# google/lyra

Hardware: NVIDIA H100
Metric: 20ms-frame encode+decode throughput (frames/s) @16kHz (higher is better)
Workload: dtype f32+i8 (decoder fp32 GEMMs: split tf32 on tensor cores)

## Files before the change

lyra_b200/csrc/kernel_prims.cuh:

```cuda
#pragma once

#include "device_compat.h"
#include "net_params.h"

namespace lyra_b200 {

template <typename T>
__device__ __forceinline__ const T* BlobPtr(const uint8_t* blob, uint32_t off) {
  return reinterpret_cast<const T*>(blob + off);
}

__device__ __forceinline__ float LeakyRelu(float v) { return fmaxf(v, __fmul_rn(v, 0.3f)); }

__device__ __forceinline__ int QuantizeF32(float v, float scale, int zp) {
  int q = (int)roundf(__fdiv_rn(v, scale)) + zp;
  q = q < -128 ? -128 : (q > 127 ? 127 : q);
  return q;
}
__device__ __forceinline__ float DequantizeI8(int q, float scale, int zp) { return __fmul_rn(scale, (float)(q - zp)); }

__device__ __forceinline__ int Mbqm(int x, int qm, int shift) {
  const int left = shift > 0 ? shift : 0, right = shift > 0 ? 0 : -shift;
  const long long ab = (long long)(int)((unsigned)x << left) * (long long)qm;
  const int hi = (int)((ab + (1ll << 30)) >> 31);
// ... 225 lines not shown
    const int tr0 = valid0 ? m0 / S : T_out - 1, tr1 = valid1 ? m1 / S : T_out - 1;
    const int s0 = m0 % S, s1 = m1 % S;
    const int grp = (nt0 * 8) / CoutG;
    const uint32_t* pa0 = A + (size_t)(grp * CinG4) * ldA + (rowA0 + tr0 * row_stride) * S + s0;
    const uint32_t* pa1 = A + (size_t)(grp * CinG4) * ldA + (rowA0 + tr1 * row_stride) * S + s1;
    const uint2* wp = Wf + (size_t)nt0 * 32 + lane;
    const size_t ks_stride = (size_t)NTILES * 32;
    int acc[NTW][4];
#pragma unroll
    for (int j = 0; j < NTW; ++j) { acc[j][0] = 0; acc[j][1] = 0; acc[j][2] = 0; acc[j][3] = 0; }
    uint2 bf[PD][NTW];
#pragma unroll
    for (int p = 0; p < PD; ++p)
      if (p < KS) {
#pragma unroll
        for (int j = 0; j < NTW; ++j) bf[p][j] = __ldg(wp + p * ks_stride + j * 32);
      }
    for (int ks0 = 0; ks0 < KS; ks0 += PD) {
#pragma unroll
      for (int p = 0; p < PD; ++p) {
        const int ks = ks0 + p;
        if (ks < KS) {
          const int kw = ks * 8, tap = kw / CinG4, kw0 = kw - tap * CinG4;
          const size_t off = (size_t)(kw0 + t4) * ldA + tap * S;
          uint32_t a[4];
          a[0] = pa0[off]; a[1] = pa1[off]; a[2] = pa0[off + 4 * (size_t)ldA]; a[3] = pa1[off + 4 * (size_t)ldA];
#pragma unroll
          for (int j = 0; j < NTW; ++j) {
            const uint32_t b[2] = {bf[p][j].x, bf[p][j].y};
            lyra_mma_s8_16x8x32(acc[j], a, b);
          }
          if (ks + PD < KS) {
#pragma unroll
            for (int j = 0; j < NTW; ++j) bf[p][j] = __ldg(wp + (size_t)(ks + PD) * ks_stride + j * 32);
          }
        }
      }
    }
    const bool even = (t4 & 1) == 0;
#pragma unroll
    for (int j = 0; j < NTW; ++j) {
      const int r0 = __shfl_xor_sync(0xffffffffu, even ? acc[j][2] : acc[j][0], 1);
      const int r1 = __shfl_xor_sync(0xffffffffu, even ? acc[j][3] : acc[j][1], 1);
      int out[1][4];
      if (even) { out[0][0] = acc[j][0]; out[0][1] = acc[j][1]; out[0][2] = r0; out[0][3] = r1; }
      else { out[0][0] = r0; out[0][1] = r1; out[0][2] = acc[j][2]; out[0][3] = acc[j][3]; }
      const int n4 = (nt0 + j) * 8 + (t4 >> 1) * 4;
      if (even ? valid0 : valid1) epi(even ? tr0 : tr1, even ? s0 : s1, n4, out);
    }
  }
  __syncthreads();
}

__host__ __device__ constexpr int PadLd(int x) {
  while (!(x % 4 == 0 && (x % 32 == 8 || x % 32 == 24))) ++x;
  return x;
}

__device__ __forceinline__ void SplitTf32(float x, uint32_t& hi, uint32_t& lo) {
  hi = __float_as_uint(x) & 0xffffe000u;
  lo = __float_as_uint(__fsub_rn(x, __uint_as_float(hi)));
}

template <int S, int NT, int WTM, int WTN, bool SYNC_EPI, typename Epi>
__device__ __forceinline__ void GemmTf32Mma(const float* A, int ldA, int rowA0, int row_stride, int ntaps, int CinG,
                                            int groups, int T_out, int N, const float2* __restrict__ Wf, Epi epi) {
  constexpr int PD = 8;
  constexpr int NW = NT / 32;
  const int lane = (int)threadIdx.x & 31, warp = (int)threadIdx.x >> 5, g = lane >> 2, t4 = lane & 3;
  const int M = T_out * S, MT = (M + 15) / 16, MTW = (MT + WTM - 1) / WTM, NTILES = N / 8, NWT = MTW * (NTILES / WTN);
  const int KS = ntaps * CinG / 8, CoutG = N / groups;
  const size_t ks_stride = (size_t)NTILES * 32;
  float acc[WTM][WTN][4];
  int tr[WTM][2], sr[WTM][2];
  bool vr[WTM][2];
  int nt0 = 0;

  auto kloop = [&](int wt) {
    const int mtb = (wt % MTW) * WTM;
    nt0 = (wt / MTW) * WTN;
    const int grp = (nt0 * 8) / CoutG;
    const float* pa[WTM][2];
#pragma unroll
    for (int i = 0; i < WTM; ++i)
#pragma unroll
      for (int h = 0; h < 2; ++h) {
        const int m = (mtb + i) * 16 + g + 8 * h;
        vr[i][h] = m < M;
        tr[i][h] = vr[i][h] ? m / S : T_out - 1;
        sr[i][h] = m % S;
        pa[i][h] = A + (size_t)(grp * CinG) * ldA + (rowA0 + tr[i][h] * row_stride) * S + sr[i][h];
      }
#pragma unroll
    for (int i = 0; i < WTM; ++i)
#pragma unroll
      for (int j = 0; j < WTN; ++j) { acc[i][j][0] = 0.0f; acc[i][j][1] = 0.0f; acc[i][j][2] = 0.0f; acc[i][j][3] = 0.0f; }
    const float2* wp = Wf + (size_t)nt0 * 32 + lane;
    float2 bf[PD][WTN];
#pragma unroll
    for (int p = 0; p < PD; ++p)
      if (p < KS) {
#pragma unroll
        for (int j = 0; j < WTN; ++j) bf[p][j] = __ldg(wp + p * ks_stride + j * 32);
      }
    for (int ks0 = 0; ks0 < KS; ks0 += PD) {
#pragma unroll
// ... 238 lines not shown
```

lyra_b200/csrc/net_kernels.cuh:

```cuda
#pragma once

#include <type_traits>

#include "kernel_prims.cuh"

namespace lyra_b200 {

constexpr int kTileStreams = 8;

struct EncStateA {
  static constexpr int kFirst = 0;
  static constexpr int kRing0 = 48, kRing1 = kRing0 + 64 * 2, kRing2 = kRing1 + 64 * 6;
  static constexpr int kDown0 = kRing2 + 64 * 18;
  static constexpr int kUnits = kDown0 + 64 * 5;
  static constexpr int kT = 20;
};
struct EncStateB {
  static constexpr int kRing0 = 0, kRing1 = 128 * 2, kRing2 = kRing1 + 128 * 6;
  static constexpr int kDown1 = kRing2 + 128 * 18;
  static constexpr int kRingM = kDown1 + 128 * 2;
  static constexpr int kRingQ0 = kRingM + 256 * 2;
  static constexpr int kRingQ1 = kRingQ0 + 64 * 6;
  static constexpr int kDown2 = kRingQ1 + 64 * 18;
  static constexpr int kBott = kDown2 + 64 * 2;
// ... 144 lines not shown
    auto epi2 = [&](int t, int s0, int n0, auto& acc) {
      constexpr int TMx = sizeof(acc) / sizeof(acc[0]), TNx = sizeof(acc[0]) / sizeof(float);
#pragma unroll
      for (int j = 0; j < TNx; ++j) {
        const float b = b2[n0 + j];
        float* o = u + (size_t)(n0 + j) * ldu + (row0u + t) * S + s0;
#pragma unroll
        for (int i = 0; i < TMx; ++i) {
          const float v = __fadd_rn(__fadd_rn(acc[i][j], b), o[i]);
          o[i] = last ? LeakyRelu(v) : v;
        }
      }
    };
    if constexpr (TC)
      GemmTf32Mma<S, NT, WTM, WTN, false>(d, ldd, 0, 1, 1, C / groups2, groups2, T, C, BlobPtr<float2>(blob, p.pw2.wf), epi2);
    else
      GemmF32Tap<S, NT, TM, TN2, KC, WM, false, STG>(d, ldd, 0, 1, 1, C / groups2, groups2, T, C, BlobPtr<float>(blob, p.pw2.w), wbuf, true, after, epi2);
  }
}

template <int S, int NT, int TM, int TN1, int TN2, int WM, int KC, int C, int T, bool TC = false, int LDD = T * S, int WTM = 1, int WTN = 1,
          int STG = kStages>
__device__ __forceinline__ void ResUnitsF32x3(const uint8_t* blob, const ResF32* p3, float* u, int ldu, int row0u, float* d, int groups2,
                                              float* ring0, const int* n18, const int* active, float* wbuf, const WNext& after) {
#pragma unroll 1
  for (int i = 0; i < 3; ++i) {
    const ResF32& p = p3[i];
    const int dil = i == 0 ? 1 : (i == 1 ? 3 : 9);
    float* ring = ring0 + (size_t)(i == 0 ? 0 : (i == 1 ? 2 : 8)) * C * S;
    const WNext nx = i < 2 ? NextF32(BlobPtr<float>(blob, p3[i + 1].pw1.w), KC, C, C, nullptr, STG) : after;
    ResUnitF32<S, NT, TM, TN1, TN2, WM, KC, C, T, 0, TC, LDD, WTM, WTN, STG>(blob, p, u, ldu, row0u, d, groups2, ring, n18, active, wbuf, i == 2, nx,
                                                                       dil);
  }
}

struct RequantLutPack {
  const int* bias;
  const int* mult;
  const int* shift;
  const int8_t* lut;
  int out_zp;
  __device__ __forceinline__ RequantLutPack(const uint8_t* blob, const GemmI8& g, const LReluQ& lr)
      : bias(BlobPtr<int>(blob, g.bias)), mult(BlobPtr<int>(blob, g.mult)), shift(BlobPtr<int>(blob, g.shift)),
        lut(BlobPtr<int8_t>(blob, lr.lut)), out_zp(g.out_zp) {}
  __device__ __forceinline__ uint32_t operator()(const int (&acc)[1][4], int n0) const {
    const RequantP4 rq = LoadRequant4(bias, mult, shift, n0);
    int q[4];
#pragma unroll
    for (int j = 0; j < 4; ++j) q[j] = lut[RequantI8(acc[0][j], rq.b[j], rq.m[j], rq.s[j], out_zp) + 128];
    return PackI8x4(q[0], q[1], q[2], q[3]);
  }
};

template <int S, int NT, int PDI, typename Params>
__device__ __forceinline__ void MixedUnitPw2I8(const uint8_t* blob, const Params& P, const uint32_t* hq, const float* u,
                                               uint32_t* resq, uint32_t* aq, int lda, int row0a) {
  constexpr int LQ2 = PadLd(2 * S), LD2 = 2 * S;
  const int* bias = BlobPtr<int>(blob, P.m_pw2.bias);
  const int* mult = BlobPtr<int>(blob, P.m_pw2.mult);
  const int* shift = BlobPtr<int>(blob, P.m_pw2.shift);
  const int8_t* lut = BlobPtr<int8_t>(blob, P.m_lr2.lut);
  const QuantP dq = P.m_dq, q2 = P.m_q2;
  const int out_zp = P.m_pw2.out_zp;
  GemmI8Mma<S, NT, 4, PDI>(hq, LQ2, 0, 1, 1, 64, 4, 2, 256, BlobPtr<uint2>(blob, P.m_pw2.w),
    [&](int t, int s, int n0, int (&acc)[1][4]) {
      const RequantP4 rq = LoadRequant4(bias, mult, shift, n0);
      int r[4], a[4];
#pragma unroll
      for (int j = 0; j < 4; ++j) {
        const int q = RequantI8(acc[0][j], rq.b[j], rq.m[j], rq.s[j], out_zp);
        const float v = __fadd_rn(DequantizeI8(q, dq.scale, dq.zp), u[(size_t)(n0 + j) * LD2 + t * S + s]);
        r[j] = QuantizeF32(v, q2.scale, q2.zp);
        a[j] = lut[r[j] + 128];
      }
      resq[(size_t)(n0 / 4) * LQ2 + t * S + s] = PackI8x4(r[0], r[1], r[2], r[3]);
      aq[(size_t)(n0 / 4) * lda + (row0a + t) * S + s] = PackI8x4(a[0], a[1], a[2], a[3]);
    });
}

template <int S, int NT, int DIL, int PDI = kI8Pd>
__device__ __forceinline__ void ResUnitI8(const uint8_t* blob, const ResI8& p, uint32_t* aq, int lda, int row0a,
                                          uint32_t* resq, uint32_t* dq8, uint32_t* hq, uint32_t* ring,
                                          const int* n18, const int* active, int dil_rt = DIL) {
  constexpr int T = kResI8Rows, C = 256, LD = PadLd(T * S);
  constexpr int NTW = 4;
  if (n18[S] >= 0) {
    if constexpr (DIL != 0) DwI8RingFast<S, NT, C, T, DIL>(aq, lda, row0a, dq8, LD, blob, p.dw, ring, n18[S], active);
    else if (dil_rt == 3) DwI8RingFast<S, NT, C, T, 3>(aq, lda, row0a, dq8, LD, blob, p.dw, ring, n18[S], active);
    else DwI8RingFast<S, NT, C, T, 9>(aq, lda, row0a, dq8, LD, blob, p.dw, ring, n18[S], active);
  } else {
    DwI8Ring<S, NT>(aq, lda, row0a, dq8, LD, C, T, dil_rt, blob, p.dw, ring, n18, active);
  }
  {
    const RequantLutPack epi(blob, p.pw1, p.lr1);
    GemmI8Mma<S, NT, NTW, PDI>(dq8, LD, 0, 1, 1, C, 1, T, C, BlobPtr<uint2>(blob, p.pw1.w),
      [&](int t, int s, int n0, int (&acc)[1][4]) { hq[(size_t)(n0 / 4) * LD + t * S + s] = epi(acc, n0); });
  }
  {
    const int* bias = BlobPtr<int>(blob, p.pw2.bias);
    const int* mult = BlobPtr<int>(blob, p.pw2.mult);
    const int* shift = BlobPtr<int>(blob, p.pw2.shift);
    const int* l1 = BlobPtr<int>(blob, p.add.lut1);
    const int* l2 = BlobPtr<int>(blob, p.add.lut2);
    const int8_t* lut = BlobPtr<int8_t>(blob, p.lr2.lut);
    const int out_zp = p.pw2.out_zp, m3 = p.add.m3, s3 = p.add.s3, add_zp = p.add.out_zp;
    GemmI8Mma<S, NT, NTW, PDI>(hq, LD, 0, 1, 1, C / 4, 4, T, C, BlobPtr<uint2>(blob, p.pw2.w),
      [&](int t, int s, int n0, int (&acc)[1][4]) {
        const RequantP4 rq = LoadRequant4(bias, mult, shift, n0);
        const size_t ro = (size_t)(n0 / 4) * LD + t * S + s;
        const uint32_t rw = resq[ro];
        int r[4], a[4];
#pragma unroll
        for (int j = 0; j < 4; ++j) {
          const int q = RequantI8(acc[0][j], rq.b[j], rq.m[j], rq.s[j], out_zp);
          r[j] = ClampI8(Mbqm(l1[q + 128] + l2[UnpackI8(rw, j) + 128], m3, s3) + add_zp);
          a[j] = lut[r[j] + 128];
        }
        resq[ro] = PackI8x4(r[0], r[1], r[2], r[3]);
        aq[(size_t)(n0 / 4) * lda + (row0a + t) * S + s] = PackI8x4(a[0], a[1], a[2], a[3]);
      });
  }
}

template <int S, int NT, int PDI = kI8Pd>
__device__ __forceinline__ void ResUnitsI8x2(const uint8_t* blob, const ResI8* p2, uint32_t* aq, int lda, int row0a,
                                             uint32_t* resq, uint32_t* dq8, uint32_t* hq, uint32_t* ring0,
                                             const int* n18, const int* active) {
#pragma unroll 1
  for (int i = 0; i < 2; ++i)
    ResUnitI8<S, NT, 0, PDI>(blob, p2[i], aq, lda, row0a, resq, dq8, hq, ring0 + (size_t)(i ? 64 * 6 : 0) * S, n18, active, i ? 9 : 3);
}

struct EncA {
  static constexpr int S = kTileStreams;
  static constexpr int NT = 320;
  static constexpr int TN = 4;
  static constexpr int kMinBlocks = 2;
  static constexpr int LDU = 25 * S, LDD = 20 * S;
  static constexpr int kStgDown = 5;
  static constexpr int DTM = 8, DTN = 4;
  static constexpr int kSmemU = 0;
  static constexpr int kSmemD = kSmemU + 64 * LDU * 4;
  static constexpr int kSmemW = kSmemD + 64 * LDD * 4;
  static constexpr int kSmemI = kSmemW + kStages * 16 * 64 * 4;
  static constexpr int kSmemBytes = kSmemI + 3 * S * 4 + 16;
  static_assert(391 * S <= 64 * LDD, "first-layer input (368 rows + 23 skew rows) must fit in the d buffer");
};

__global__ void __launch_bounds__(EncA::NT, EncA::kMinBlocks)
EncoderKernelA(const uint8_t* __restrict__ blob, EncoderParams P, TileIo io, const int16_t* __restrict__ pcm,
               float* __restrict__ state, int* __restrict__ n18g, float* __restrict__ mid) {
  using L = EncA;
  constexpr int S = L::S, NT = L::NT;
  unsigned char* smem = LYRA_DYN_SMEM();
  float* u = reinterpret_cast<float*>(smem + L::kSmemU);
  float* d = reinterpret_cast<float*>(smem + L::kSmemD);
  float* wbuf = reinterpret_cast<float*>(smem + L::kSmemW);
  int* slot = reinterpret_cast<int*>(smem + L::kSmemI);
  int* active = slot + S;
  int* n18 = active + S;
  int tile;
  InitWeightPipe<NT>();
  if (!BeginTile<S>(io, n18g, slot, state, EncStateA::kUnits, tile)) return;
  float* st = state + (size_t)tile * EncStateA::kUnits * S;
  const int tid = (int)threadIdx.x;
  IssuePrologue<NT>(wbuf, NextF32(BlobPtr<float>(blob, P.first.w), 16, 64, 64));

  float* X = d;
  BatchedLoop<NT, 2, float>(48 * S, [&](int i) { return st[EncStateA::kFirst * S + i]; },
                            [&](int i, float v) { const int r = i / S; X[(r + (r >> 4)) * S + i % S] = v; });
  BatchedLoop<NT, 8, float>(320 * S,
    [&](int i) { const int s = i / 320, k = i % 320; return active[s] ? (float)pcm[(size_t)slot[s] * 320 + k] * (1.0f / 32768.0f) : 0.0f; },
    [&](int i, float v) { const int s = i / 320, k = i % 320; X[(48 + k + ((48 + k) >> 4)) * S + s] = v; });
  BatchedLoop<NT, 8, float>(64 * 5 * S, [&](int i) { return st[EncStateA::kDown0 * S + i]; },
                            [&](int i, float v) { const int c = i / (5 * S), r = i % (5 * S); u[(size_t)c * L::LDU + r] = v; });
  __syncthreads();
  for (int i = tid; i < 48 * S; i += NT)
    if (active[i % S]) { const int r = 320 + i / S; st[EncStateA::kFirst * S + i] = X[(r + (r >> 4)) * S + i % S]; }
  {
    const float* b = BlobPtr<float>(blob, P.first.bias);
    GemmF32Tap<S, NT, 8, L::TN, 16, 4, true>(X, 0, 0, 17, 64, 1, 1, 20, 64, BlobPtr<float>(blob, P.first.w), wbuf, true,
      NextF32(BlobPtr<float>(blob, P.r0[0].pw1.w), 16, 64, 64),
      [&](int t, int s0, int n0, float (&acc)[8][L::TN]) {
#pragma unroll
        for (int j = 0; j < L::TN; ++j) {
          float* o = u + (size_t)(n0 + j) * L::LDU + (5 + t) * S + s0;
#pragma unroll
          for (int i = 0; i < 8; ++i) o[i] = __fadd_rn(acc[i][j], b[n0 + j]);
        }
      });
  }
  static_assert(EncStateA::kRing1 == EncStateA::kRing0 + 64 * 2 && EncStateA::kRing2 == EncStateA::kRing1 + 64 * 6, "ring blocks back to back");
  ResUnitsF32x3<S, NT, 8, L::TN, L::TN, 4, 16, 64, EncStateA::kT>(blob, P.r0, u, L::LDU, 5, d, 1, st + (size_t)EncStateA::kRing0 * S, n18, active, wbuf,
                                                       NextF32(BlobPtr<float>(blob, P.down0.w), 16, 128, 640, d, L::kStgDown));
  StoreCarriedRows<S, NT, 64, 5>(st, EncStateA::kDown0, u, L::LDU, 20, active);
  {
    const float* b = BlobPtr<float>(blob, P.down0.bias);
    float* out = mid + (size_t)tile * 128 * 4 * S;
    static_assert(L::kStgDown * 16 * 128 * 4 <= 64 * L::LDD * 4, "simpleconv weight ring must fit in d");
    constexpr int DTM = L::DTM, DTN = L::DTN;
    GemmF32Tap<S, NT, DTM, DTN, 16, 4, false, L::kStgDown>(u, L::LDU, 0, 5, 10, 64, 1, 4, 128, BlobPtr<float>(blob, P.down0.w), d, true, NoNext(),
      [&](int t, int s0, int n0, float (&acc)[DTM][DTN]) {
#pragma unroll
        for (int j = 0; j < DTN; ++j) {
          float* o = out + ((size_t)(n0 + j) * 4 + t) * S + s0;
#pragma unroll
          for (int i = 0; i < DTM; ++i) o[i] = __fadd_rn(acc[i][j], b[n0 + j]);
        }
      });
  }
  AdvanceHopCounters<S>(n18g, tile, active, n18);
}

struct EncB {
  static constexpr int S = kTileStreams;
  static constexpr int NT = 256;
  static constexpr int kMinBlocks = 3;
  static constexpr int TM = 8;
  static constexpr int TN = 4;
  static constexpr int WM4 = 4 * S / TM >= 4 ? 4 : 4 * S / TM;
  static constexpr int WM2 = 2 * S / TM >= 4 ? 4 : 2 * S / TM;
  static constexpr int WM1 = 1 * S / TM >= 4 ? 4 : 1 * S / TM;
  static constexpr int LD1 = 6 * S;
  static constexpr int LQ2 = PadLd(2 * S), LQA = PadLd(4 * S), LQB = PadLd(3 * S);
  static constexpr int kRA = 0;
  static constexpr int kRABytes = kMax(kMax(128 * LD1 * 4, 256 * 2 * S * 4), 64 * LQA * 4 + 128 * LQB * 4);
  static constexpr int kRB = kRA + kRABytes;
  static constexpr int kRBBytes = kMax(128 * 4 * S * 4, 256 * 2 * S * 4);
  static constexpr int kRC = kRB + kRBBytes;
  static constexpr int kW = kRC + 64 * LQ2 * 4;
  static constexpr int kStg = 3;
  static constexpr int kWBytes = kMax(kStg * 8 * 256 * 4, 2 * 64 * LQ2 * 4);
  static constexpr int kI8Pd = 4;
  static constexpr int kI = kW + kWBytes;
  static constexpr int kSmemBytes = kI + 3 * S * 4 + 16;
};

__global__ void __launch_bounds__(EncB::NT, EncB::kMinBlocks)
EncoderKernelB(const uint8_t* __restrict__ blob, EncoderParams P, TileIo io, const float* __restrict__ mid,
               float* __restrict__ state, int* __restrict__ n18g, float* __restrict__ features) {
  using L = EncB;
  constexpr int S = L::S, NT = L::NT;
  constexpr int TM = L::TM, TN = L::TN;
  unsigned char* smem = LYRA_DYN_SMEM();
  constexpr int LQ2 = L::LQ2, LQA = L::LQA, LQB = L::LQB;
  float* u1 = reinterpret_cast<float*>(smem + L::kRA);
  float* d2 = reinterpret_cast<float*>(smem + L::kRA);
  uint32_t* aq = reinterpret_cast<uint32_t*>(smem + L::kRA);
  uint32_t* bq = aq + 64 * LQA;
  float* d1 = reinterpret_cast<float*>(smem + L::kRB);
  float* u2 = reinterpret_cast<float*>(smem + L::kRB);
  uint32_t* hq = reinterpret_cast<uint32_t*>(smem + L::kRC);
  float* wbuf = reinterpret_cast<float*>(smem + L::kW);
  uint32_t* dq8 = reinterpret_cast<uint32_t*>(smem + L::kW);
  uint32_t* resq = dq8 + 64 * LQ2;
  int* slot = reinterpret_cast<int*>(smem + L::kI);
  int* active = slot + S;
  int* n18 = active + S;
  int tile;
  InitWeightPipe<NT>();
  if (!BeginTile<S>(io, n18g, slot, state, EncStateB::kUnits, tile)) return;
  float* st = state + (size_t)tile * EncStateB::kUnits * S;
  uint32_t* stw = reinterpret_cast<uint32_t*>(st);
  IssuePrologue<NT>(wbuf, NextF32(BlobPtr<float>(blob, P.r1[0].pw1.w), 16, 128, 128, nullptr, L::kStg));

  {
    const float* in = mid + (size_t)tile * 128 * 4 * S;
    BatchedLoop<NT, 4, float4>(128 * S, [&](int i) { return reinterpret_cast<const float4*>(in)[i]; },
      [&](int i, float4 v) { const int c = i / S, r = (i % S) * 4; *reinterpret_cast<float4*>(u1 + (size_t)c * L::LD1 + 2 * S + r) = v; });
    BatchedLoop<NT, 8, float>(128 * 2 * S, [&](int i) { return st[EncStateB::kDown1 * S + i]; },
      [&](int i, float v) { const int c = i / (2 * S), r = i % (2 * S); u1[(size_t)c * L::LD1 + r] = v; });
  }
  __syncthreads();
  static_assert(EncStateB::kRing1 == EncStateB::kRing0 + 128 * 2 && EncStateB::kRing2 == EncStateB::kRing1 + 128 * 6, "ring blocks back to back");
  ResUnitsF32x3<S, NT, TM, TN, TN, L::WM4, 16, 128, EncStateB::kT1, false, 4 * S, 1, 1, L::kStg>(
      blob, P.r1, u1, L::LD1, 2, d1, 2, st + (size_t)EncStateB::kRing0 * S, n18, active, wbuf,
      NextF32(BlobPtr<float>(blob, P.down1.w), 8, 256, 256, wbuf, L::kStg));
  StoreCarriedRows<S, NT, 128, 2>(st, EncStateB::kDown1, u1, L::LD1, 4, active);
  {
    const float* b = BlobPtr<float>(blob, P.down1.bias);
    GemmF32Tap<S, NT, TM, TN, 8, L::WM2, false, L::kStg>(u1, L::LD1, 0, 2, 4, 64, 2, 2, 256, BlobPtr<float>(blob, P.down1.w), wbuf, true,
      NextF32(BlobPtr<float>(blob, P.m_pw1.w), 8, 256, 256, wbuf, L::kStg),
      [&](int t, int s0, int n0, float (&acc)[TM][TN]) {
#pragma unroll
        for (int j = 0; j < TN; ++j) {
          float* o = u2 + (size_t)(n0 + j) * 2 * S + t * S + s0;
#pragma unroll
          for (int i = 0; i < TM; ++i) o[i] = __fadd_rn(acc[i][j], b[n0 + j]);
        }
      });
  }
  constexpr int LD2 = 2 * S;
  if (n18[S] >= 0)
    DwF32RingFast<S, NT, 256, EncStateB::kT2, 1>(u2, LD2, 0, d2, LD2, BlobPtr<float>(blob, P.m_dw.w), BlobPtr<float>(blob, P.m_dw.bias),
                                    st + (size_t)EncStateB::kRingM * S, n18[S], active);
  else
    DwF32Ring<S, NT>(u2, LD2, 0, d2, LD2, 256, EncStateB::kT2, 1, BlobPtr<float>(blob, P.m_dw.w), BlobPtr<float>(blob, P.m_dw.bias),
                     st + (size_t)EncStateB::kRingM * S, n18, active);
  {
    const float* b = BlobPtr<float>(blob, P.m_pw1.bias);
    const int8_t* lut = BlobPtr<int8_t>(blob, P.m_lr1.lut);
    const QuantP q1 = P.m_q1;
    static_assert(TN == 4, "the epilogue packs one word of four channels per (row, stream)");
    GemmF32Tap<S, NT, TM, TN, 8, L::WM2, false, L::kStg>(d2, LD2, 0, 1, 1, 256, 1, 2, 256, BlobPtr<float>(blob, P.m_pw1.w), wbuf, true,
      NoNext(),
      [&](int t, int s0, int n0, float (&acc)[TM][TN]) {
#pragma unroll
        for (int i = 0; i < TM; ++i) {
          int q[TN];
#pragma unroll
          for (int j = 0; j < TN; ++j) q[j] = lut[QuantizeF32(__fadd_rn(acc[i][j], b[n0 + j]), q1.scale, q1.zp) + 128];
          hq[(size_t)(n0 / 4) * LQ2 + t * S + s0 + i] = PackI8x4(q[0], q[1], q[2], q[3]);
        }
      });
  }
  MixedUnitPw2I8<S, NT, L::kI8Pd>(blob, P, hq, u2, resq, aq, LQA, 2);
  static_assert(EncStateB::kRingQ1 == EncStateB::kRingQ0 + 64 * 6, "ring blocks back to back");
  ResUnitsI8x2<S, NT, L::kI8Pd>(blob, P.q, aq, LQA, 2, resq, dq8, hq, stw + (size_t)EncStateB::kRingQ0 * S, n18, active);
  BatchedLoop<NT, 4, uint32_t>(64 * 2 * S, [&](int i) { return stw[EncStateB::kDown2 * S + i]; },
    [&](int i, uint32_t v) { const int c = i / (2 * S), r = i % (2 * S); aq[(size_t)c * LQA + r] = v; });
  BatchedLoop<NT, 8, uint32_t>(128 * 2 * S, [&](int i) { return stw[EncStateB::kBott * S + i]; },
    [&](int i, uint32_t v) { const int c = i / (2 * S), r = i % (2 * S); bq[(size_t)c * LQB + r] = v; });
  __syncthreads();
  StoreCarriedRows<S, NT, 64, 2>(stw, EncStateB::kDown2, aq, LQA, 2, active);
  {
    const RequantLutPack epi(blob, P.down2, P.down2_lr);
    GemmI8Mma<S, NT, 8, L::kI8Pd>(aq, LQA, 0, 2, 4, 64, 4, 1, 512, BlobPtr<uint2>(blob, P.down2.w),
      [&](int, int s, int n0, int (&acc)[1][4]) { bq[(size_t)(n0 / 4) * LQB + 2 * S + s] = epi(acc, n0); });
  }
  StoreCarriedRows<S, NT, 128, 2>(stw, EncStateB::kBott, bq, LQB, 1, active);
  {
    const int* bias = BlobPtr<int>(blob, P.bott.bias);
    const int* mult = BlobPtr<int>(blob, P.bott.mult);
    const int* shift = BlobPtr<int>(blob, P.bott.shift);
    const QuantP dq = P.out_dq;
    const int out_zp = P.bott.out_zp;
    GemmI8Mma<S, NT, 1, L::kI8Pd>(bq, LQB, 0, 1, 3, 128, 4, 1, 64, BlobPtr<uint2>(blob, P.bott.w),
      [&](int t, int s, int n0, int (&acc)[1][4]) {
        const RequantP4 rq = LoadRequant4(bias, mult, shift, n0);
        (void)t;
        if (!active[s]) return;
        float* o = features + (size_t)slot[s] * 64 + n0;
#pragma unroll
        for (int j = 0; j < 4; ++j)
          o[j] = DequantizeI8(RequantI8(acc[0][j], rq.b[j], rq.m[j], rq.s[j], out_zp), dq.scale, dq.zp);
      });
  }
  AdvanceHopCounters<S>(n18g, tile, active, n18);
}

template <bool TC = false>
struct DecC {
  static constexpr int S = kTileStreams;
  static constexpr int NT = 256;
  static constexpr int kMinBlocks = 3;
  static constexpr int kI8Pd = 2;
  static constexpr int TM = 8;
  static constexpr int TN = 4;
  static constexpr int WM4 = 4 * S / TM >= 4 ? 4 : 4 * S / TM;
  static constexpr int WM2 = 2 * S / TM >= 4 ? 4 : 2 * S / TM;
  static constexpr int WM1 = 1 * S / TM >= 4 ? 4 : 1 * S / TM;
  static constexpr int LQ2 = PadLd(2 * S), LQA = PadLd(4 * S), LQB = PadLd(3 * S);
  static constexpr int kF = 0;
  static constexpr int kXq = kF + 64 * 3 * S * 4;
  static constexpr int LD1 = TC ? PadLd(4 * S) : 4 * S;
  static constexpr int RWM = 2, RWN = 2;
  static_assert(!TC || ((4 * S + 31) / 32) * (16 / RWN) <= NT / 32, "decoder_1: one warp tile per warp");
  static constexpr int kR1Bytes = kMax(kMax(64 * 3 * S * 4 + 128 * LQB * 4, 64 * LQA * 4), 128 * LD1 * 4);
  static constexpr int kU = kF + kR1Bytes;
  static constexpr int kW = kU + 256 * 2 * S * 4;
  static constexpr int kWBytes = kMax(kStages * 4 * 512 * 4, 3 * 64 * LQ2 * 4);
  static constexpr int kI = kW + kWBytes;
  static constexpr int kSmemBytes = kI + 3 * S * 4 + 16;
};

template <bool TC>
__global__ void __launch_bounds__(DecC<TC>::NT, DecC<TC>::kMinBlocks)
DecoderKernelC(const uint8_t* __restrict__ blob, DecoderParams P, TileIo io,
               const float* __restrict__ features, float* __restrict__ state, int* __restrict__ n18g,
               float* __restrict__ mid) {
  using L = DecC<TC>;
  constexpr int S = L::S, NT = L::NT;
  constexpr int TM = L::TM, TN = L::TN;
  unsigned char* smem = LYRA_DYN_SMEM();
  float* F = reinterpret_cast<float*>(smem + L::kF);
  uint32_t* xq = reinterpret_cast<uint32_t*>(smem + L::kXq);
  float* u = reinterpret_cast<float*>(smem + L::kU);
  float* u1 = u;
  constexpr int LQ2 = L::LQ2, LQA = L::LQA, LQB = L::LQB;
  uint32_t* aq = reinterpret_cast<uint32_t*>(smem + L::kF);
  float* d1 = reinterpret_cast<float*>(smem + L::kF);
  float* wbuf = reinterpret_cast<float*>(smem + L::kW);
  uint32_t* hq = reinterpret_cast<uint32_t*>(smem + L::kW);
  uint32_t* dq8 = hq + 64 * LQ2;
  uint32_t* resq = dq8 + 64 * LQ2;
  int* slot = reinterpret_cast<int*>(smem + L::kI);
  int* active = slot + S;
  int* n18 = active + S;
  int tile;
  InitWeightPipe<NT>();
  if (!BeginTile<S>(io, n18g, slot, state, DecStateC::kUnits, tile)) return;
  uint32_t* stw = reinterpret_cast<uint32_t*>(state) + (size_t)tile * DecStateC::kUnits * S;
  float* st = reinterpret_cast<float*>(stw);
  const int tid = (int)threadIdx.x;
  constexpr int LD2 = 2 * S;
  const UpI8& up0 = P.up0;
  const UpI8& up1 = P.up1;
  IssuePrologue<NT>(wbuf, NextF32(BlobPtr<float>(blob, P.bott.w), 4, 512, 48));

  BatchedLoop<NT, 4, float>(64 * 2 * S, [&](int i) { return st[DecStateC::kBott * S + i]; },
    [&](int i, float v) { const int c = i / (2 * S), r = i % (2 * S); F[(size_t)c * 3 * S + r] = v; });
  BatchedLoop<NT, 2, float>(64 * S, [&](int i) { const int s = i / 64, c = i % 64; return active[s] ? features[(size_t)slot[s] * 64 + c] : 0.0f; },
    [&](int i, float v) { const int s = i / 64, c = i % 64; F[(size_t)c * 3 * S + 2 * S + s] = v; });
  BatchedLoop<NT, 4, float4>(256 * 2 * S / 4, [&](int i) { return reinterpret_cast<const float4*>(st + (size_t)DecStateC::kUp0 * S)[i]; },
    [&](int i, float4 v) { reinterpret_cast<float4*>(u)[i] = v; });
  {
    const uint32_t pad = PackI8x4(P.bott_q.zp, P.bott_q.zp, P.bott_q.zp, P.bott_q.zp);
    for (int i = tid; i < 128 * S; i += NT) { const int c = i / S, s = i % S; xq[(size_t)c * LQB + s] = pad; xq[(size_t)c * LQB + 2 * S + s] = pad; }
  }
  __syncthreads();
  StoreCarriedRows<S, NT, 64, 2>(st, DecStateC::kBott, F, 3 * S, 1, active);
  {
    const float* b = BlobPtr<float>(blob, P.bott.bias);
    const QuantP q = P.bott_q;
    GemmF32Tap<S, NT, TM, 4, 4, L::WM1, false>(F, 3 * S, 0, 1, 3, 16, 4, 1, 512, BlobPtr<float>(blob, P.bott.w), wbuf, true,
      NoNext(),
      [&](int t, int s0, int n0, float (&acc)[TM][4]) {
        (void)t;
#pragma unroll
        for (int i = 0; i < TM; ++i) {
          int v[4];
#pragma unroll
          for (int j = 0; j < 4; ++j) v[j] = QuantizeF32(LeakyRelu(__fadd_rn(acc[i][j], b[n0 + j])), q.scale, q.zp);
          xq[(size_t)(n0 / 4) * LQB + S + s0 + i] = PackI8x4(v[0], v[1], v[2], v[3]);
        }
      });
  }
  {
    const int* bias = BlobPtr<int>(blob, up0.g.bias);
    const int* mult = BlobPtr<int>(blob, up0.g.mult);
    const int* shift = BlobPtr<int>(blob, up0.g.shift);
    float* tail = st + (size_t)DecStateC::kUp0 * S;
    GemmI8Mma<S, NT, 8>(xq, LQB, 0, 1, 2, 128, 4, 2, 512, BlobPtr<uint2>(blob, up0.g.w),
      [&](int q, int s, int n0, int (&acc)[1][4]) {
        const RequantP4 rq = LoadRequant4(bias, mult, shift, n0);
        const int g = n0 / 128, r = (n0 % 128) / 64;
        const float* bf = BlobPtr<float>(blob, up0.bias_f32[g]);
#pragma unroll
        for (int j = 0; j < 4; ++j) {
          const int co = (n0 + j) % 64, ch = g * 64 + co;
          const int qv = RequantI8(acc[0][j], rq.b[j], rq.m[j], rq.s[j], up0.out_zp[g]);
          const float f = DequantizeI8(qv, up0.dq[g].scale, up0.dq[g].zp);
          if (q == 0) {
            float* o = u + (size_t)ch * LD2 + r * S + s;
            *o = __fadd_rn(f, *o);
          } else if (active[s]) {
            tail[((size_t)ch * 2 + r) * S + s] = __fsub_rn(__fadd_rn(f, 0.0f), bf[co]);
          }
        }
      });
  }
  {
    const QuantP q = P.up0_q;
    for (int i = tid; i < 64 * 2 * S; i += NT) {
      const int c4 = i / (2 * S), r = i % (2 * S);
      int v[4];
#pragma unroll
      for (int b = 0; b < 4; ++b) v[b] = QuantizeF32(LeakyRelu(u[(size_t)(c4 * 4 + b) * LD2 + r]), q.scale, q.zp);
      aq[(size_t)c4 * LQA + S + r] = PackI8x4(v[0], v[1], v[2], v[3]);
    }
  }
  __syncthreads();
  if (n18[S] >= 0) DwI8RingFast<S, NT, 256, DecStateC::kT0, 1>(aq, LQA, 1, dq8, LQ2, blob, P.m_dw, stw + (size_t)DecStateC::kRingM * S, n18[S], active);
  else DwI8Ring<S, NT>(aq, LQA, 1, dq8, LQ2, 256, DecStateC::kT0, 1, blob, P.m_dw, stw + (size_t)DecStateC::kRingM * S, n18, active);
  {
    const RequantLutPack epi(blob, P.m_pw1, P.m_lr1);
    GemmI8Mma<S, NT, 4, L::kI8Pd>(dq8, LQ2, 0, 1, 1, 256, 1, 2, 256, BlobPtr<uint2>(blob, P.m_pw1.w),
      [&](int t, int s, int n0, int (&acc)[1][4]) { hq[(size_t)(n0 / 4) * LQ2 + t * S + s] = epi(acc, n0); });
  }
  MixedUnitPw2I8<S, NT, L::kI8Pd>(blob, P, hq, u, resq, aq, LQA, 1);
  static_assert(DecStateC::kRingQ1 == DecStateC::kRingQ0 + 64 * 6, "ring blocks back to back");
  ResUnitsI8x2<S, NT, L::kI8Pd>(blob, P.q, aq, LQA, 1, resq, dq8, hq, stw + (size_t)DecStateC::kRingQ0 * S, n18, active);
  {
    const uint32_t pad = PackI8x4(up1.g.in_zp, up1.g.in_zp, up1.g.in_zp, up1.g.in_zp);
    for (int i = tid; i < 64 * S; i += NT) { const int c = i / S, s = i % S; aq[(size_t)c * LQA + s] = pad; aq[(size_t)c * LQA + 3 * S + s] = pad; }
    BatchedLoop<NT, 8, float>(128 * 4 * S,
      [&](int i) { const int c = i / (4 * S), r = i % (4 * S); return r < 2 * S ? st[DecStateC::kUp1 * S + (size_t)c * 2 * S + r] : 0.0f; },
      [&](int i, float v) { u1[i] = v; });
  }
  __syncthreads();
  {
    const int* bias = BlobPtr<int>(blob, up1.g.bias);
    const int* mult = BlobPtr<int>(blob, up1.g.mult);
    const int* shift = BlobPtr<int>(blob, up1.g.shift);
    float* tail = st + (size_t)DecStateC::kUp1 * S;
    if (!TC) IssuePrologue<NT>(wbuf, NextF32(BlobPtr<float>(blob, P.r1[0].pw1.w), 16, 128, 128));
    GemmI8Mma<S, NT, 8>(aq, LQA, 0, 1, 2, 128, 2, 3, 256, BlobPtr<uint2>(blob, up1.g.w),
      [&](int q, int s, int n0, int (&acc)[1][4]) {
        const RequantP4 rq = LoadRequant4(bias, mult, shift, n0);
        const int g = n0 / 128, r = (n0 % 128) / 64;
        const float* bf = BlobPtr<float>(blob, up1.bias_f32[g]);
#pragma unroll
        for (int j = 0; j < 4; ++j) {
          const int co = (n0 + j) % 64, ch = g * 64 + co;
          const int qv = RequantI8(acc[0][j], rq.b[j], rq.m[j], rq.s[j], up1.out_zp[g]);
          const float f = DequantizeI8(qv, up1.dq[g].scale, up1.dq[g].zp);
          if (q < 2) {
            float* o = u1 + (size_t)ch * 4 * S + (2 * q + r) * S + s;
            *o = __fadd_rn(f, *o);
          } else if (active[s]) {
            tail[((size_t)ch * 2 + r) * S + s] = __fsub_rn(__fadd_rn(f, 0.0f), bf[co]);
          }
        }
      });
  }
  static_assert(DecStateC::kRing1 == DecStateC::kRing0 + 128 * 2 && DecStateC::kRing2 == DecStateC::kRing1 + 128 * 6, "ring blocks back to back");
  ResUnitsF32x3<S, NT, TM, TN, TN, L::WM4, 16, 128, DecStateC::kT1, TC, L::LD1, L::RWM, L::RWN>(
      blob, P.r1, u1, 4 * S, 0, d1, 2, st + (size_t)DecStateC::kRing0 * S, n18, active, wbuf, NoNext());
  {
    float* out = mid + (size_t)tile * 128 * 4 * S;
    for (int i = tid; i < 128 * 4 * S; i += NT) out[i] = u1[i];
  }
  AdvanceHopCounters<S>(n18g, tile, active, n18);
}

struct DecD {
  static constexpr int S = kTileStreams;
  static constexpr int NT = 320;
  static constexpr int TN = 4;
  static constexpr int kMinBlocks = 2;
  static constexpr int TNU = 5;
  static constexpr int TNL = 2;
  static constexpr int WML = 4;
  static constexpr int WMU = 1;
  static constexpr int KCU = 8;
  static constexpr int LDU = 26 * S, LDD = 20 * S, LDX = 6 * S;
  static constexpr int kU = 0;
  static constexpr int kD = kU + 64 * LDU * 4;
  static constexpr int kW = kD + 64 * LDD * 4;
  static constexpr int kWBytes = kStages * 16 * 64 * 4 + 2048;
  static constexpr int kSl = kW + kWBytes;
  static_assert(128 * 6 * S * 4 + kStages * KCU * 320 * 4 <= 64 * LDD * 4 + kWBytes, "decoder_2/simple ring must fit behind X");
  static constexpr int kI = kSl + 48 * S * 4;
  static constexpr int kSmemBytes = kI + 3 * S * 4 + 16;
  static_assert(128 * LDX <= 64 * LDD, "X must fit in d");
  static_assert(S * 320 * 2 <= 64 * LDD * 4, "PCM staging must fit in d");
};

__global__ void __launch_bounds__(DecD::NT, DecD::kMinBlocks)
DecoderKernelD(const uint8_t* __restrict__ blob, DecoderParams P, TileIo io, const float* __restrict__ mid,
// ... 96 lines not shown
```

Before: 4.194 million.

## Stream int8 GEMM weights through a bulk-copy mbarrier ring with cross-layer prefetch

Adds GemmI8Ring, an int8 MMA GEMM that stages weight chunks into a shared-memory ring using bulk async copies and full/empty mbarriers. Each GEMM prefetches the next layer's weight prologue, chaining encoder and decoder int8 layers, where weights were previously read straight from global memory. Shared memory is reallocated: dq8 and resq move into the bq region and the decoder gets a separate quantizer ring. The aim is to hide weight-fetch latency, at the cost of per-chunk barrier synchronization and more complex smem aliasing.

Result: no change. 4.207 million (median of 6 runs) (+0.3%).

```diff
diff --git a/lyra_b200/csrc/kernel_prims.cuh b/lyra_b200/csrc/kernel_prims.cuh
--- a/lyra_b200/csrc/kernel_prims.cuh
+++ b/lyra_b200/csrc/kernel_prims.cuh
@@ -301,6 +301,85 @@
   __syncthreads();
 }
 
+__device__ __forceinline__ WNext NextI8(const uint2* w, int N, int KS, int kpc, int chn, void* ring, int stages) {
+  return WNext{w, kpc * chn * 64, (KS / kpc) * (N / 8 / chn), ring, stages};
+}
+template <int S, int NT, int NTW, int KPC, int CHN, int STG, typename Epi>
+__device__ __forceinline__ void GemmI8Ring(const uint32_t* A, int ldA, int rowA0, int row_stride, int ntaps, int CinG,
+                                           int groups, int T_out, int N, const uint2* __restrict__ Wf, uint2* ring,
+                                           const WNext& nxt, Epi epi) {
+  static_assert(STG >= 2 && STG <= kMaxStages && CHN % NTW == 0, "ring shape");
+  constexpr int CW = KPC * CHN * 32;
+  const int lane = (int)threadIdx.x & 31, warp = (int)threadIdx.x >> 5, g = lane >> 2, t4 = lane & 3;
+  const int M = T_out * S, MT = (M + 15) / 16, NTILES = N / 8, NWT = MT * (NTILES / NTW);
+  const int CinG4 = CinG / 4, KS = ntaps * CinG4 / 8, CoutG = N / groups;
+  const int CPK = NTILES / CHN, nchunks = (KS / KPC) * CPK;
+  if (NWT != NT / 32 || KS % KPC != 0 || NTILES % CHN != 0 || (KPC > 1 && CPK != 1) || nchunks < STG - 1) LYRA_TRAP();
+  WeightPipe* pipe = GetWeightPipe();
+  const int set = pipe->cur;
+  if (threadIdx.x == 0) InitPipeSet(pipe, set ^ 1, NT / 32);
+  const int mt = warp % MT, nt0 = (warp / MT) * NTW;
+  const int m0 = mt * 16 + g, m1 = m0 + 8;
+  const bool valid0 = m0 < M, valid1 = m1 < M;
+  const int tr0 = valid0 ? m0 / S : T_out - 1, tr1 = valid1 ? m1 / S : T_out - 1;
+  const int s0 = m0 % S, s1 = m1 % S;
+  const int grp = (nt0 * 8) / CoutG;
+  const uint32_t* pa0 = A + (size_t)(grp * CinG4) * ldA + (rowA0 + tr0 * row_stride) * S + s0;
+  const uint32_t* pa1 = A + (size_t)(grp * CinG4) * ldA + (rowA0 + tr1 * row_stride) * S + s1;
+  const int myc = nt0 / CHN;
+  int acc[NTW][4];
+#pragma unroll
+  for (int j = 0; j < NTW; ++j) { acc[j][0] = 0; acc[j][1] = 0; acc[j][2] = 0; acc[j][3] = 0; }
+  for (int c = 0; c < nchunks; ++c) {
+    if (threadIdx.x == 0) {
+      const int ci = c + STG - 1;
+      if (ci < nchunks) {
+        const int si = ci % STG;
+        if (ci >= STG) lyra_mbar_wait(&pipe->empty[set][si], (unsigned)((ci / STG - 1) & 1));
+        lyra_bulk_g2s(ring + (size_t)si * CW, Wf + (size_t)ci * CW, (unsigned)CW * 8u, &pipe->full[set][si]);
+      }
+    }
+    const int st = c % STG;
+    lyra_mbar_wait(&pipe->full[set][st], (unsigned)((c / STG) & 1));
+    if (c % CPK == myc) {
+      const uint2* bp = ring + (size_t)st * CW + (nt0 - myc * CHN) * 32 + lane;
+#pragma unroll
+      for (int kk = 0; kk < KPC; ++kk) {
+        const int kw = ((c / CPK) * KPC + kk) * 8, tap = kw / CinG4, kw0 = kw - tap * CinG4;
+        const size_t off = (size_t)(kw0 + t4) * ldA + tap * S;
+        uint32_t a[4];
+        a[0] = pa0[off]; a[1] = pa1[off]; a[2] = pa0[off + 4 * (size_t)ldA]; a[3] = pa1[off + 4 * (size_t)ldA];
+#pragma unroll
+        for (int j = 0; j < NTW; ++j) {
+          const uint2 bw = bp[(kk * CHN + j) * 32];
+          const uint32_t b[2] = {bw.x, bw.y};
+          lyra_mma_s8_16x8x32(acc[j], a, b);
+        }
+      }
+    }
+    __syncwarp();
+    if (lane == 0) lyra_mbar_arrive(&pipe->empty[set][st]);
+  }
+  lyra_fence_proxy_async();
+  __syncthreads();
+  if (threadIdx.x == 0) {
+    if (nxt.w != nullptr) IssuePrologueSet(pipe, set ^ 1, nxt.ring ? nxt.ring : ring, nxt.w, nxt.chunk_words, nxt.nchunks, nxt.stages);
+    pipe->cur = set ^ 1;
+  }
+  const bool even = (t4 & 1) == 0;
+#pragma unroll
+  for (int j = 0; j < NTW; ++j) {
+    const int r0 = __shfl_xor_sync(0xffffffffu, even ? acc[j][2] : acc[j][0], 1);
+    const int r1 = __shfl_xor_sync(0xffffffffu, even ? acc[j][3] : acc[j][1], 1);
+    int out[1][4];
+    if (even) { out[0][0] = acc[j][0]; out[0][1] = acc[j][1]; out[0][2] = r0; out[0][3] = r1; }
+    else { out[0][0] = r0; out[0][1] = r1; out[0][2] = acc[j][2]; out[0][3] = acc[j][3]; }
+    const int n4 = (nt0 + j) * 8 + (t4 >> 1) * 4;
+    if (even ? valid0 : valid1) epi(even ? tr0 : tr1, even ? s0 : s1, n4, out);
+  }
+  __syncthreads();
+}
+
 __host__ __device__ constexpr int PadLd(int x) {
   while (!(x % 4 == 0 && (x % 32 == 8 || x % 32 == 24))) ++x;
   return x;
diff --git a/lyra_b200/csrc/net_kernels.cuh b/lyra_b200/csrc/net_kernels.cuh
--- a/lyra_b200/csrc/net_kernels.cuh
+++ b/lyra_b200/csrc/net_kernels.cuh
@@ -220,9 +220,21 @@
   }
 };
 
-template <int S, int NT, int PDI, typename Params>
+template <int S, int NT, int NTW, int PDI, int RSTG, int KPC, int CHN, typename Epi>
+__device__ __forceinline__ void GemmI8(const uint32_t* A, int ldA, int rowA0, int row_stride, int ntaps, int CinG, int groups,
+                                       int T_out, int N, const uint2* __restrict__ Wf, uint2* ring, const WNext& nxt, Epi epi) {
+  if constexpr (RSTG > 0)
+    GemmI8Ring<S, NT, NTW, KPC, CHN, RSTG>(A, ldA, rowA0, row_stride, ntaps, CinG, groups, T_out, N, Wf, ring, nxt, epi);
+  else
+    GemmI8Mma<S, NT, NTW, PDI>(A, ldA, rowA0, row_stride, ntaps, CinG, groups, T_out, N, Wf, epi);
+}
+__device__ __forceinline__ WNext NextI8x256(const uint8_t* blob, uint32_t w, int CinG, uint2* ring, int stages) {
+  return NextI8(BlobPtr<uint2>(blob, w), 256, CinG / 32, 1, 32, ring, stages);
+}
+
+template <int S, int NT, int PDI, int RSTG, typename Params>
 __device__ __forceinline__ void MixedUnitPw2I8(const uint8_t* blob, const Params& P, const uint32_t* hq, const float* u,
-                                               uint32_t* resq, uint32_t* aq, int lda, int row0a) {
+                                               uint32_t* resq, uint32_t* aq, int lda, int row0a, uint2* ring, const WNext& after) {
   constexpr int LQ2 = PadLd(2 * S), LD2 = 2 * S;
   const int* bias = BlobPtr<int>(blob, P.m_pw2.bias);
   const int* mult = BlobPtr<int>(blob, P.m_pw2.mult);
@@ -230,7 +242,7 @@
   const int8_t* lut = BlobPtr<int8_t>(blob, P.m_lr2.lut);
   const QuantP dq = P.m_dq, q2 = P.m_q2;
   const int out_zp = P.m_pw2.out_zp;
-  GemmI8Mma<S, NT, 4, PDI>(hq, LQ2, 0, 1, 1, 64, 4, 2, 256, BlobPtr<uint2>(blob, P.m_pw2.w),
+  GemmI8<S, NT, 4, PDI, RSTG, 1, 32>(hq, LQ2, 0, 1, 1, 64, 4, 2, 256, BlobPtr<uint2>(blob, P.m_pw2.w), ring, after,
     [&](int t, int s, int n0, int (&acc)[1][4]) {
       const RequantP4 rq = LoadRequant4(bias, mult, shift, n0);
       int r[4], a[4];
@@ -246,10 +258,10 @@
     });
 }
 
-template <int S, int NT, int DIL, int PDI = kI8Pd>
+template <int S, int NT, int DIL, int PDI = kI8Pd, int RSTG = 0>
 __device__ __forceinline__ void ResUnitI8(const uint8_t* blob, const ResI8& p, uint32_t* aq, int lda, int row0a,
                                           uint32_t* resq, uint32_t* dq8, uint32_t* hq, uint32_t* ring,
-                                          const int* n18, const int* active, int dil_rt = DIL) {
+                                          const int* n18, const int* active, uint2* wring, const WNext& after, int dil_rt = DIL) {
   constexpr int T = kResI8Rows, C = 256, LD = PadLd(T * S);
   constexpr int NTW = 4;
   if (n18[S] >= 0) {
@@ -261,7 +273,8 @@
   }
   {
     const RequantLutPack epi(blob, p.pw1, p.lr1);
-    GemmI8Mma<S, NT, NTW, PDI>(dq8, LD, 0, 1, 1, C, 1, T, C, BlobPtr<uint2>(blob, p.pw1.w),
+    GemmI8<S, NT, NTW, PDI, RSTG, 1, 32>(dq8, LD, 0, 1, 1, C, 1, T, C, BlobPtr<uint2>(blob, p.pw1.w), wring,
+      NextI8x256(blob, p.pw2.w, C / 4, wring, RSTG),
       [&](int t, int s, int n0, int (&acc)[1][4]) { hq[(size_t)(n0 / 4) * LD + t * S + s] = epi(acc, n0); });
   }
   {
@@ -272,7 +285,7 @@
     const int* l2 = BlobPtr<int>(blob, p.add.lut2);
     const int8_t* lut = BlobPtr<int8_t>(blob, p.lr2.lut);
     const int out_zp = p.pw2.out_zp, m3 = p.add.m3, s3 = p.add.s3, add_zp = p.add.out_zp;
-    GemmI8Mma<S, NT, NTW, PDI>(hq, LD, 0, 1, 1, C / 4, 4, T, C, BlobPtr<uint2>(blob, p.pw2.w),
+    GemmI8<S, NT, NTW, PDI, RSTG, 1, 32>(hq, LD, 0, 1, 1, C / 4, 4, T, C, BlobPtr<uint2>(blob, p.pw2.w), wring, after,
       [&](int t, int s, int n0, int (&acc)[1][4]) {
         const RequantP4 rq = LoadRequant4(bias, mult, shift, n0);
         const size_t ro = (size_t)(n0 / 4) * LD + t * S + s;
@@ -290,13 +303,16 @@
   }
 }
 
-template <int S, int NT, int PDI = kI8Pd>
+template <int S, int NT, int PDI = kI8Pd, int RSTG = 0>
 __device__ __forceinline__ void ResUnitsI8x2(const uint8_t* blob, const ResI8* p2, uint32_t* aq, int lda, int row0a,
                                              uint32_t* resq, uint32_t* dq8, uint32_t* hq, uint32_t* ring0,
-                                             const int* n18, const int* active) {
+                                             const int* n18, const int* active, uint2* wring, const WNext& after) {
 #pragma unroll 1
-  for (int i = 0; i < 2; ++i)
-    ResUnitI8<S, NT, 0, PDI>(blob, p2[i], aq, lda, row0a, resq, dq8, hq, ring0 + (size_t)(i ? 64 * 6 : 0) * S, n18, active, i ? 9 : 3);
+  for (int i = 0; i < 2; ++i) {
+    const WNext nx = i == 0 ? NextI8x256(blob, p2[1].pw1.w, 256, wring, RSTG) : after;
+    ResUnitI8<S, NT, 0, PDI, RSTG>(blob, p2[i], aq, lda, row0a, resq, dq8, hq, ring0 + (size_t)(i ? 64 * 6 : 0) * S, n18, active,
+                                   wring, nx, i ? 9 : 3);
+  }
 }
 
 struct EncA {
@@ -398,8 +414,10 @@
   static constexpr int kRC = kRB + kRBBytes;
   static constexpr int kW = kRC + 64 * LQ2 * 4;
   static constexpr int kStg = 3;
-  static constexpr int kWBytes = kMax(kStg * 8 * 256 * 4, 2 * 64 * LQ2 * 4);
-  static constexpr int kI8Pd = 4;
+  static constexpr int kI8Stg = 3;
+  static constexpr int kI8Chunk = 8192;
+  static constexpr int kWBytes = kMax(kStg * 8 * 256 * 4, kI8Stg * kI8Chunk);
+  static_assert(2 * 64 * LQ2 <= 128 * LQB, "dq8 and resq fit where bq goes");
   static constexpr int kI = kW + kWBytes;
   static constexpr int kSmemBytes = kI + 3 * S * 4 + 16;
 };
@@ -420,12 +438,14 @@
   float* u2 = reinterpret_cast<float*>(smem + L::kRB);
   uint32_t* hq = reinterpret_cast<uint32_t*>(smem + L::kRC);
   float* wbuf = reinterpret_cast<float*>(smem + L::kW);
-  uint32_t* dq8 = reinterpret_cast<uint32_t*>(smem + L::kW);
+  uint2* wring = reinterpret_cast<uint2*>(smem + L::kW);
+  uint32_t* dq8 = bq;
   uint32_t* resq = dq8 + 64 * LQ2;
   int* slot = reinterpret_cast<int*>(smem + L::kI);
   int* active = slot + S;
   int* n18 = active + S;
   int tile;
+  constexpr int RSTG = L::kI8Stg;
   InitWeightPipe<NT>();
   if (!BeginTile<S>(io, n18g, slot, state, EncStateB::kUnits, tile)) return;
   float* st = state + (size_t)tile * EncStateB::kUnits * S;
@@ -471,7 +491,7 @@
     const QuantP q1 = P.m_q1;
     static_assert(TN == 4, "the epilogue packs one word of four channels per (row, stream)");
     GemmF32Tap<S, NT, TM, TN, 8, L::WM2, false, L::kStg>(d2, LD2, 0, 1, 1, 256, 1, 2, 256, BlobPtr<float>(blob, P.m_pw1.w), wbuf, true,
-      NoNext(),
+      NextI8x256(blob, P.m_pw2.w, 64, wring, RSTG),
       [&](int t, int s0, int n0, float (&acc)[TM][TN]) {
 #pragma unroll
         for (int i = 0; i < TM; ++i) {
@@ -482,9 +502,11 @@
         }
       });
   }
-  MixedUnitPw2I8<S, NT, L::kI8Pd>(blob, P, hq, u2, resq, aq, LQA, 2);
+  MixedUnitPw2I8<S, NT, 0, RSTG>(blob, P, hq, u2, resq, aq, LQA, 2, wring, NextI8x256(blob, P.q[0].pw1.w, 256, wring, RSTG));
   static_assert(EncStateB::kRingQ1 == EncStateB::kRingQ0 + 64 * 6, "ring blocks back to back");
-  ResUnitsI8x2<S, NT, L::kI8Pd>(blob, P.q, aq, LQA, 2, resq, dq8, hq, stw + (size_t)EncStateB::kRingQ0 * S, n18, active);
+  static_assert(L::kI8Chunk == 32 * 32 * 8 && L::kI8Chunk == 4 * 8 * 32 * 8, "int8 chunk shapes");
+  ResUnitsI8x2<S, NT, 0, RSTG>(blob, P.q, aq, LQA, 2, resq, dq8, hq, stw + (size_t)EncStateB::kRingQ0 * S, n18, active, wring,
+                                      NextI8(BlobPtr<uint2>(blob, P.down2.w), 512, 8, 1, 32, wring, RSTG));
   BatchedLoop<NT, 4, uint32_t>(64 * 2 * S, [&](int i) { return stw[EncStateB::kDown2 * S + i]; },
     [&](int i, uint32_t v) { const int c = i / (2 * S), r = i % (2 * S); aq[(size_t)c * LQA + r] = v; });
   BatchedLoop<NT, 8, uint32_t>(128 * 2 * S, [&](int i) { return stw[EncStateB::kBott * S + i]; },
@@ -493,7 +515,8 @@
   StoreCarriedRows<S, NT, 64, 2>(stw, EncStateB::kDown2, aq, LQA, 2, active);
   {
     const RequantLutPack epi(blob, P.down2, P.down2_lr);
-    GemmI8Mma<S, NT, 8, L::kI8Pd>(aq, LQA, 0, 2, 4, 64, 4, 1, 512, BlobPtr<uint2>(blob, P.down2.w),
+    GemmI8<S, NT, 8, 0, RSTG, 1, 32>(aq, LQA, 0, 2, 4, 64, 4, 1, 512, BlobPtr<uint2>(blob, P.down2.w), wring,
+      NextI8(BlobPtr<uint2>(blob, P.bott.w), 64, 12, 4, 8, wring, RSTG),
       [&](int, int s, int n0, int (&acc)[1][4]) { bq[(size_t)(n0 / 4) * LQB + 2 * S + s] = epi(acc, n0); });
   }
   StoreCarriedRows<S, NT, 128, 2>(stw, EncStateB::kBott, bq, LQB, 1, active);
@@ -503,7 +526,7 @@
     const int* shift = BlobPtr<int>(blob, P.bott.shift);
     const QuantP dq = P.out_dq;
     const int out_zp = P.bott.out_zp;
-    GemmI8Mma<S, NT, 1, L::kI8Pd>(bq, LQB, 0, 1, 3, 128, 4, 1, 64, BlobPtr<uint2>(blob, P.bott.w),
+    GemmI8<S, NT, 1, 0, RSTG, 4, 8>(bq, LQB, 0, 1, 3, 128, 4, 1, 64, BlobPtr<uint2>(blob, P.bott.w), wring, NoNext(),
       [&](int t, int s, int n0, int (&acc)[1][4]) {
         const RequantP4 rq = LoadRequant4(bias, mult, shift, n0);
         (void)t;
@@ -529,6 +552,7 @@
   static constexpr int WM2 = 2 * S / TM >= 4 ? 4 : 2 * S / TM;
   static constexpr int WM1 = 1 * S / TM >= 4 ? 4 : 1 * S / TM;
   static constexpr int LQ2 = PadLd(2 * S), LQA = PadLd(4 * S), LQB = PadLd(3 * S);
+  static constexpr int kI8Stg = TC ? 0 : 3;
   static constexpr int kF = 0;
   static constexpr int kXq = kF + 64 * 3 * S * 4;
   static constexpr int LD1 = TC ? PadLd(4 * S) : 4 * S;
@@ -540,6 +564,9 @@
   static constexpr int kWBytes = kMax(kStages * 4 * 512 * 4, 3 * 64 * LQ2 * 4);
   static constexpr int kI = kW + kWBytes;
   static constexpr int kSmemBytes = kI + 3 * S * 4 + 16;
+  static constexpr int kI8Chunk = 8192;
+  static constexpr int kQ = kF + 64 * LQA * 4;
+  static_assert(kI8Stg * kI8Chunk <= kWBytes && kQ + kI8Stg * kI8Chunk <= kW, "int8 weight rings");
 };
 
 template <bool TC>
@@ -562,10 +589,13 @@
   uint32_t* hq = reinterpret_cast<uint32_t*>(smem + L::kW);
   uint32_t* dq8 = hq + 64 * LQ2;
   uint32_t* resq = dq8 + 64 * LQ2;
+  uint2* wring = reinterpret_cast<uint2*>(smem + L::kW);
+  uint2* qring = reinterpret_cast<uint2*>(smem + L::kQ);
   int* slot = reinterpret_cast<int*>(smem + L::kI);
   int* active = slot + S;
   int* n18 = active + S;
   int tile;
+  constexpr int RSTG = L::kI8Stg;
   InitWeightPipe<NT>();
   if (!BeginTile<S>(io, n18g, slot, state, DecStateC::kUnits, tile)) return;
   uint32_t* stw = reinterpret_cast<uint32_t*>(state) + (size_t)tile * DecStateC::kUnits * S;
@@ -592,7 +622,7 @@
     const float* b = BlobPtr<float>(blob, P.bott.bias);
     const QuantP q = P.bott_q;
     GemmF32Tap<S, NT, TM, 4, 4, L::WM1, false>(F, 3 * S, 0, 1, 3, 16, 4, 1, 512, BlobPtr<float>(blob, P.bott.w), wbuf, true,
-      NoNext(),
+      RSTG > 0 ? NextI8(BlobPtr<uint2>(blob, up0.g.w), 512, 8, 1, 32, wring, RSTG) : NoNext(),
       [&](int t, int s0, int n0, float (&acc)[TM][4]) {
         (void)t;
 #pragma unroll
@@ -609,7 +639,7 @@
     const int* mult = BlobPtr<int>(blob, up0.g.mult);
     const int* shift = BlobPtr<int>(blob, up0.g.shift);
     float* tail = st + (size_t)DecStateC::kUp0 * S;
-    GemmI8Mma<S, NT, 8>(xq, LQB, 0, 1, 2, 128, 4, 2, 512, BlobPtr<uint2>(blob, up0.g.w),
+    GemmI8<S, NT, 8, kI8Pd, RSTG, 1, 32>(xq, LQB, 0, 1, 2, 128, 4, 2, 512, BlobPtr<uint2>(blob, up0.g.w), wring, NoNext(),
       [&](int q, int s, int n0, int (&acc)[1][4]) {
         const RequantP4 rq = LoadRequant4(bias, mult, shift, n0);
         const int g = n0 / 128, r = (n0 % 128) / 64;
@@ -646,9 +676,11 @@
     GemmI8Mma<S, NT, 4, L::kI8Pd>(dq8, LQ2, 0, 1, 1, 256, 1, 2, 256, BlobPtr<uint2>(blob, P.m_pw1.w),
       [&](int t, int s, int n0, int (&acc)[1][4]) { hq[(size_t)(n0 / 4) * LQ2 + t * S + s] = epi(acc, n0); });
   }
-  MixedUnitPw2I8<S, NT, L::kI8Pd>(blob, P, hq, u, resq, aq, LQA, 1);
+  MixedUnitPw2I8<S, NT, L::kI8Pd, 0>(blob, P, hq, u, resq, aq, LQA, 1, nullptr, NoNext());
   static_assert(DecStateC::kRingQ1 == DecStateC::kRingQ0 + 64 * 6, "ring blocks back to back");
-  ResUnitsI8x2<S, NT, L::kI8Pd>(blob, P.q, aq, LQA, 1, resq, dq8, hq, stw + (size_t)DecStateC::kRingQ0 * S, n18, active);
+  if (RSTG > 0) IssuePrologue<NT>(qring, NextI8x256(blob, P.q[0].pw1.w, 256, qring, RSTG));
+  ResUnitsI8x2<S, NT, L::kI8Pd, RSTG>(blob, P.q, aq, LQA, 1, resq, dq8, hq, stw + (size_t)DecStateC::kRingQ0 * S, n18, active, qring,
+                                      NoNext());
   {
     const uint32_t pad = PackI8x4(up1.g.in_zp, up1.g.in_zp, up1.g.in_zp, up1.g.in_zp);
     for (int i = tid; i < 64 * S; i += NT) { const int c = i / S, s = i % S; aq[(size_t)c * LQA + s] = pad; aq[(size_t)c * LQA + 3 * S + s] = pad; }
@@ -662,8 +694,9 @@
     const int* mult = BlobPtr<int>(blob, up1.g.mult);
     const int* shift = BlobPtr<int>(blob, up1.g.shift);
     float* tail = st + (size_t)DecStateC::kUp1 * S;
-    if (!TC) IssuePrologue<NT>(wbuf, NextF32(BlobPtr<float>(blob, P.r1[0].pw1.w), 16, 128, 128));
-    GemmI8Mma<S, NT, 8>(aq, LQA, 0, 1, 2, 128, 2, 3, 256, BlobPtr<uint2>(blob, up1.g.w),
+    if (RSTG > 0) IssuePrologue<NT>(wring, NextI8(BlobPtr<uint2>(blob, up1.g.w), 256, 8, 1, 32, wring, RSTG));
+    GemmI8<S, NT, 8, kI8Pd, RSTG, 1, 32>(aq, LQA, 0, 1, 2, 128, 2, 3, 256, BlobPtr<uint2>(blob, up1.g.w), wring,
+      TC ? NoNext() : NextF32(BlobPtr<float>(blob, P.r1[0].pw1.w), 16, 128, 128, wbuf),
       [&](int q, int s, int n0, int (&acc)[1][4]) {
         const RequantP4 rq = LoadRequant4(bias, mult, shift, n0);
         const int g = n0 / 128, r = (n0 % 128) / 64;
```
